# compbioproj-cdna-to-genome-map-align/gmap-2024

Measured on AMD Instinct MI355X. Metric: aligned cDNA reads/sec (2 kb, GRCh38) at 1/2/4/8 MI355X; DP HBM GB/s vs peak, higher is better.
Workload: dtype int32

## Files before the change

gmap-2024_amd/csrc/dp_device.h:

```cpp
#pragma once
#include <hip/hip_runtime.h>
#include <stdint.h>


#include "gmapdp_internal.h"
#include "../../include/gmapdp.h"
#include "me_device.h"

namespace gmapdp {


constexpr int kSent = (int)0x80000000;

__device__ __forceinline__ int dpp_wave_shl1(int x, int fill) {
  return __builtin_amdgcn_update_dpp(fill, x, 0x130, 0xf, 0xf, false);
}
__device__ __forceinline__ int dpp_wave_shl1_zero(int x) {
  return __builtin_amdgcn_update_dpp(0, x, 0x130, 0xf, 0xf, true);
}
__device__ __forceinline__ int dpp_wave_shr1(int x, int fill) {
  return __builtin_amdgcn_update_dpp(fill, x, 0x138, 0xf, 0xf, false);
}
__device__ __forceinline__ int dpp_wave_shr1_zero(int x) {
  return __builtin_amdgcn_update_dpp(0, x, 0x138, 0xf, 0xf, true);
// ... 196 lines not shown
    const int rr = rs - j;
    const int qp = G.qpos(rr);
    const bool good = active && qp >= 0 && gp >= 0;
    const uint64_t mgood = ballot(good);
    if (good) put_pair(out, t.count + lanes_below(mgood, lane), qp, gp, 0, q[rr], '-', ' ', ' ');
    const int nw = __popcll(mgood);
    t.count += nw;
    if (!t.seen) t.lead += nw;
  }
  t.score += kQopen + dist * kQindel;
  t.nopens += 1;
  t.nindels += dist;
}

__device__ __forceinline__ void emit_genomeskip(int lane, int r, int cs, int dist, const Geo& G, bool watson,
                                                uint64_t chroffset, uint64_t chrhigh, const uint32_t* blocks,
                                                uint64_t nwords, gmapdp_pair* out, Tally& t) {
  if (dist >= kMicrointronLength) {
    if (lane == 0) put_pair(out, t.count, -1, -1, dist, ' ', ' ', ' ', ' ');
    t.count += 1;
    t.seen = true;
    return;
  }
  const int qp = G.qpos(r);
  for (int base = 0; base < dist; base += 64) {
    const int j = base + lane;
    const bool active = j < dist;
    const int gp = G.gpos(cs - j);
    const bool good = active && qp >= 0 && gp >= 0;
    const uint64_t mgood = ballot(good);
    if (good) {
      const char c2 = genomic_nt(blocks, nwords, gp, chroffset, chrhigh, watson);
      put_pair(out, t.count + lanes_below(mgood, lane), qp, gp, 0, ' ', '-', c2, c2);
    }
    const int nw = __popcll(mgood);
    t.count += nw;
    if (!t.seen) t.lead += nw;
  }
  t.score += kTopen + dist * kTindel;
  t.nopens += 1;
  t.nindels += dist;
}

__device__ __forceinline__ uint64_t wave_max_u64(uint64_t x) {
#pragma unroll
  for (int off = 32; off >= 1; off >>= 1) {
    const uint64_t y = __shfl_xor(x, off, 64);
    x = y > x ? y : x;
  }
  return x;
}
template <int S>
__device__ __forceinline__ uint64_t seg_max_u64(uint64_t x) {
#pragma unroll
  for (int off = S / 2; off >= 1; off >>= 1) {
    const uint64_t y = __shfl_xor(x, off, 64);
    x = y > x ? y : x;
  }
  return x;
}

struct BridgeCarry {
  const uint8_t* rowdi;
  const uint8_t* coldi;
  const double* rowp;
  const double* colp;
  const int8_t* isc;
  int rdist;
  struct Part* part;
  int* diag;
};
struct Part {
  double p;
  int s;
  int c;
};

__host__ __device__ inline int gg_dir_nhigh(int W) { return W <= 32 ? 0 : W <= 40 ? 1 : W <= 48 ? 2 : 4; }
struct PackedDirs {
  const uint32_t* lo;
  const uint32_t* hi;
  int W, uband, nhigh;
  __device__ uint32_t operator()(int c, int t, int r) const {
    const int k = r - c + uband;
    if (k < 0 || k >= W) return 0u;
    if (k < 32) return (lo[4 * c + t] >> k) & 1u;
    const int b = t * 8 * nhigh + (k - 32);
    return (hi[c * nhigh + (b >> 5)] >> (b & 31)) & 1u;
  }
};

template <int R, bool CARRY, int S = 64, bool PK = (S < 64), bool STORE = false, bool DPK = false, bool NB = false>
__device__ __forceinline__ void fill_band(int lane, int rlen, int glen, int lband, int uband, int open, int ext,
                                          int late, int track, const int8_t* sc, int srow, const uint8_t* gcl,
                                          uint64_t* dirs, const BridgeCarry* bc_, int& bestr, int& bestc,
                                          int gmax = 0, int* smat = nullptr, int* best_score = nullptr) {
  static_assert(S == 64 || (R == 1 && !CARRY), "segmented fills are single-word, no bridge carry");
  static_assert(!STORE || S == 64, "score matrices are stored by whole-wave fills only");
  static_assert(!DPK || (R == 1 && S == 64), "packed direction words: one-word bands");
  static_assert(!NB || S == 64, "narrow-band shifts: whole-wave fills");
  const int lk = (S == 64) ? lane : (lane & (S - 1));
  const int cend = (S == 64) ? glen : gmax;
  const int sat = kNegInf32;
  const int W = lband + uband + 1;
  const int binit = (track == 2) ? kNegInf32 : 0;
  int Hs[R], E[R], bv[R], bcol[R];
#pragma unroll
  for (int i = 0; i < R; i++) {
    const int k = lk * R + i;
    const int r = k - uband;
    int v = kNegInf32;
    if (k < W && r >= 0 && r <= rlen) v = (r == 0) ? 0 : (r <= lband ? open + r * ext : kNegInf32);
    Hs[i] = v;
    E[i] = kNegInf32;
    bv[i] = binit;
    bcol[i] = 0;
  }
  int kext[R];
#pragma unroll
  for (int i = 0; i < R; i++) kext[i] = (lk * R + i) * ext;
  int cs[R], cc[R];
  double cp[R];
#pragma unroll
  for (int i = 0; i < R; i++) {
    cs[i] = 0;
    cc[i] = 0;
    cp[i] = 0.0;
  }
  int rlen1 = rlen + 1;
  uint32_t scb = 0;
  if constexpr (CARRY && PK) {
    scb = (uint32_t)(size_t)(const __attribute__((address_space(3))) int32_t*)reinterpret_cast<const int32_t*>(sc);
    asm volatile("" : "+v"(rlen1), "+v"(scb));
  }
  int rtop_ext = -uband * ext;
  int oce = open;
  int gi_next = (S == 64) ? 0 : gcl[min(1, glen)];
  for (int c = 1; c <= cend; c++) {
    const bool colact = (S == 64) || (c <= glen);
    int gi;
    if constexpr (S == 64) {
      gi = __builtin_amdgcn_readfirstlane(gcl[c]);
    } else {
      gi = gi_next;
      gi_next = gcl[min(c + 1, glen)];
    }
    const int rtop = c - uband;
    const int rlo = rtop < 1 ? 1 : rtop;
    const int rhigh = (c + lband) < rlen ? (c + lband) : rlen;
    rtop_ext += ext;
    oce += ext;
    const int L0 = (c == 1) ? (kNegInf32 - open + 1) : (c <= uband ? oce : kNegInf32);
    const int row0 = (c <= uband) ? oce : kNegInf32;
    const int8_t* scg = PK ? sc : sc + gi * srow;
    const int gi4 = gi << 2;

    int Ein[R], Hin[R];
#pragma unroll
    for (int i = 0; i < R - 1; i++) { Ein[i] = E[i + 1]; Hin[i] = Hs[i + 1]; }
    if constexpr (NB) {
      Ein[R - 1] = dpp_wave_shl1_zero(E[0]);
      Hin[R - 1] = dpp_wave_shl1_zero(Hs[0]);
    } else {
      Ein[R - 1] = seg_shl1<S>(E[0], kNegInf32, lk);
      Hin[R - 1] = seg_shl1<S>(Hs[0], kNegInf32, lk);
    }

    int Hp[R], En[R], A[R];
    bool valid[R], eb[R], hb[R];
#pragma unroll
    for (int i = 0; i < R; i++) {
      const int k = lk * R + i;
      const int r = rtop + k;
      valid[i] = (k < W) & (r >= rlo) & (r <= rhigh) & colact;
      const int rr = (int)min((unsigned)r, (unsigned)rlen1);
      int s;
      if constexpr (!PK) s = scg[rr];
      else if constexpr (CARRY)
        s = __builtin_amdgcn_sbfe(*(const __attribute__((address_space(3))) int32_t*)(size_t)(scb + 4u * (uint32_t)rr),
                                  gi4, 4);
      else s = __builtin_amdgcn_sbfe(reinterpret_cast<const int32_t*>(sc)[rr], gi4, 4);
      const int es = Hin[i] + open;
      eb[i] = Ein[i] > es - late;
      En[i] = max(Ein[i], es) + ext;
      const int dg = Hs[i] + s;
      hb[i] = En[i] > dg - late;
      Hp[i] = max(En[i], dg);
      A[i] = valid[i] ? Hp[i] + open - rtop_ext - kext[i] : kSent;
    }
    int pre[R];
    pre[0] = A[0];
#pragma unroll
    for (int i = 1; i < R; i++) pre[i] = max(pre[i - 1], A[i]);
    const int X = seg_shr1<S>(seg_scan_max<S>(pre[R - 1]), kSent, lk);
    const int init = max(kNegInf32, L0 + open) - ((rtop > 1) ? rtop_ext - ext : 0);
    int F[R], Hun[R];
    bool vb[R];
#pragma unroll
    for (int i = 0; i < R; i++) {
      const int ex = (i == 0) ? X : max(X, pre[i - 1]);
      F[i] = rtop_ext + kext[i] + max(init, ex);
      vb[i] = F[i] > Hp[i] - late;
      Hun[i] = max(F[i], Hp[i]);
    }
    int Fup, Hup;
    if constexpr (S == 64) {
      Fup = dpp_wave_shr1_zero(F[R - 1]);
      Hup = dpp_wave_shr1_zero(Hun[R - 1]);
    } else {
      Fup = seg_shr1<S>(F[R - 1], kNegInf32, lk);
      Hup = seg_shr1<S>(Hun[R - 1], kNegInf32, lk);
    }
    uint64_t mH[R], mV[R], mE[R], mF[R];
#pragma unroll
    for (int i = 0; i < R; i++) {
      const int k = lk * R + i;
      const int r = rtop + k;
      const bool top = r == rlo;
      const int fprev = top ? kNegInf32 : ((i == 0) ? Fup : F[i - 1]);
      const int hprev = top ? L0 : ((i == 0) ? Hup : Hun[i - 1]);
      const bool fb = fprev > hprev + open - late;
      const uint64_t mvalid = ballot(valid[i]);
      mV[i] = ballot(vb[i]) & mvalid;
      mH[i] = ballot(hb[i]) & ~mV[i] & mvalid;
      mE[i] = ballot(eb[i]) & mvalid;
      mF[i] = ballot(fb) & mvalid;
      const int Hc = max(Hun[i], sat);
      if (STORE && valid[i]) smat[(size_t)c * W + k] = Hc;
      Hs[i] = valid[i] ? ((k == 0) ? Hun[i] : Hc) : ((r == 0) ? row0 : kNegInf32);
      E[i] = valid[i] ? En[i] : kNegInf32;
      const bool cand = valid[i] & ((track == 1) | ((track == 2) & (r == rlen))) & (Hc > bv[i] - late);
      bv[i] = cand ? Hc : bv[i];
      bcol[i] = cand ? c : bcol[i];
    }
    if (CARRY) {
      const BridgeCarry& B = *bc_;
      const int cdi = __builtin_amdgcn_readfirstlane(B.coldi[c]);
      const double cpc = B.colp[c];
      int ics[R], icc[R];
      double icp[R];
#pragma unroll
      for (int i = 0; i < R - 1; i++) { ics[i] = cs[i + 1]; icc[i] = cc[i + 1]; icp[i] = cp[i + 1]; }
      ics[R - 1] = dpp_wave_shl1_zero(cs[0]);
      icc[R - 1] = dpp_wave_shl1_zero(cc[0]);
      {
        const int2 v = *reinterpret_cast<const int2*>(&cp[0]);
        int2 w;
        w.x = dpp_wave_shl1_zero(v.x);
        w.y = dpp_wave_shl1_zero(v.y);
        icp[R - 1] = *reinterpret_cast<const double*>(&w);
      }
#pragma unroll
      for (int i = 0; i < R; i++) {
        const int k = lk * R + i;
        const int r = rtop + k;
        const int other = rlen - r;
        const bool inrow = (r >= 1) & (r <= rlen - 1) & (k < W);
        const bool cand = inrow & (k >= 1) & valid[i] & (c <= glen - 2) & (c < B.rdist - other);
        const int Hc = max(Hun[i], sat);
        int s = 0;
        double p = 0.0;
        if (cand) {
          s = B.isc[B.rowdi[other] & cdi] + Hc;
          p = B.rowp[other] + cpc;
        }
        const bool take = cand & ((icc[i] == 0) | (s > ics[i]) | ((s == ics[i]) & (p > icp[i])));
        cs[i] = take ? s : ics[i];
        cc[i] = take ? c + 1 : icc[i];
        cp[i] = take ? p : icp[i];
        if (inrow && k == uband) B.diag[r] = Hc;
        if (inrow && k == 0) {
          B.part[r].s = cs[i];
          B.part[r].c = cc[i] - 1;
          B.part[r].p = cp[i];
        }
      }
    }
#ifdef GMAPDP_GGX_NODIRS
    if (!CARRY)
#endif
    if constexpr (DPK) {
      if (lane == 0) {
        uint32_t* lo = reinterpret_cast<uint32_t*>(dirs);
        *reinterpret_cast<uint4*>(lo + 4 * c) = make_uint4((uint32_t)mH[0], (uint32_t)mV[0], (uint32_t)mE[0], (uint32_t)mF[0]);
        const int nh = gg_dir_nhigh(W);
        uint32_t* hi = lo + 4 * (glen + 1) + nh * c;
        const uint32_t h0 = (uint32_t)(mH[0] >> 32), h1 = (uint32_t)(mV[0] >> 32), h2 = (uint32_t)(mE[0] >> 32),
                       h3 = (uint32_t)(mF[0] >> 32);
        if (nh == 1) {
          hi[0] = (h0 & 0xffu) | ((h1 & 0xffu) << 8) | ((h2 & 0xffu) << 16) | (h3 << 24);
        } else if (nh == 2) {
          *reinterpret_cast<uint2*>(hi) = make_uint2((h0 & 0xffffu) | (h1 << 16), (h2 & 0xffffu) | (h3 << 16));
        } else if (nh == 4) {
          *reinterpret_cast<uint4*>(hi) = make_uint4(h0, h1, h2, h3);
        }
      }
    } else
    if (lane == 0) {
      uint64_t* dcol = dirs + (size_t)c * 4 * R;
#pragma unroll
      for (int i = 0; i < R; i++) {
        dcol[0 * R + i] = mH[i];
        dcol[1 * R + i] = mV[i];
        dcol[2 * R + i] = mE[i];
// ... 157 lines not shown
      bestc = 0;
    } else {
      const uint32_t rk = (uint32_t)(key >> 12) & 4095u, ck = (uint32_t)key & 4095u;
      bestr = late ? (int)rk : 4095 - (int)rk;
      bestc = late ? (int)ck : 4095 - (int)ck;
    }
  } else {
    bestr = rlen;
    bestc = glen;
  }
}

template <int R>
struct RowDirs {
  const uint64_t* dirs;
  int W, uband;
  __device__ uint32_t operator()(int c, int t, int r) const {
    const int k = r - c + uband;
    if (k < 0 || k >= W || r < 0) return 0u;
    return (uint32_t)(dirs[((size_t)c * 4 + t) * R + (r % R)] >> (r / R)) & 1u;
  }
};

template <typename DA, typename QV, typename GV>
__device__ __forceinline__ void traceback_walk(int lane, const DA& dir, int r, int c, const Geo& G, const QV& q,
                                               const QV& quc, const GV& gch, const uint8_t* __restrict__ cons,
                                               bool watson, uint64_t chroffset, uint64_t chrhigh,
                                               const uint32_t* __restrict__ blocks, uint64_t nwords,
                                               gmapdp_pair* out, Tally& t, int mode = 0) {
  while (r > 0 && c > 0) {
    const uint32_t isV = dir(c, 1, r);
    const uint32_t isH = dir(c, 0, r);
    if (!isV && isH) {
      int n = 0;
      for (int base = 0;; base += 64) {
        const int j = base + lane;
        const bool cont = (c - j >= 1) && dir(c - j, 2, r);
        const uint64_t stop = ~ballot(cont);
        if (stop) { n = base + __ffsll((long long)stop) - 1; break; }
      }
      const int dist = n + 1;
      const int c_end = (c - n - 1) > 0 ? (c - n - 1) : 0;
      emit_genomeskip(lane, r, c_end + dist, dist, G, watson, chroffset, chrhigh, blocks, nwords, out, t);
      c = c_end;
    } else if (isV) {
      int n = 0;
      for (int base = 0;; base += 64) {
        const int j = base + lane;
        const bool cont = (r - j >= 1) && dir(c, 3, r - j);
        const uint64_t stop = ~ballot(cont);
        if (stop) { n = base + __ffsll((long long)stop) - 1; break; }
      }
      const int dist = n + 1;
      const int r_end = (r - n - 1) > 0 ? (r - n - 1) : 0;
      emit_queryskip(lane, r_end + dist, c, dist, G, q, out, t);
      r = r_end;
    } else {
      int n = 0;
      for (int base = 0;; base += 64) {
        const int j = base + lane;
        const bool inrange = (c - j >= 1) && (r - j >= 1);
        const bool cont = (j == 0) || (inrange && !dir(c - j, 0, r - j) && !dir(c - j, 1, r - j));
        const uint64_t stop = ~ballot(cont && inrange);
        if (stop) { n = base + __ffsll((long long)stop) - 1; break; }
      }
      emit_diag(lane, r, c, n, G, q, quc, gch, cons, out, t);
      r -= n;
      c -= n;
    }
  }
  if ((r == 0 && c == 0) || (mode == 1 && c == 0) || (mode == 2 && r == 0)) {
  } else if (mode == 2 || (mode == 0 && c == 0)) {
    emit_queryskip(lane, r, 1, r, G, q, out, t);
  } else {
    emit_genomeskip(lane, 1, c, c, G, watson, chroffset, chrhigh, blocks, nwords, out, t);
  }
}

template <int R, typename WORD>
struct BandDirs {
  const WORD* dirs;
  int W, uband, bitoff;
  __device__ uint32_t operator()(int c, int t, int r) const {
    return dir_bit<R, WORD>(dirs, c, t, r - c + uband, W, bitoff);
  }
};

template <int R, typename WORD = uint64_t, typename QV = const char*, typename GV = const char*>
__device__ __forceinline__ void traceback_band(int lane, const WORD* dirs, int W, int uband, int r, int c,
                                               const Geo& G, const QV& q, const QV& quc, const GV& gch,
                                               const uint8_t* __restrict__ cons, bool watson, uint64_t chroffset,
                                               uint64_t chrhigh, const uint32_t* __restrict__ blocks,
                                               uint64_t nwords, gmapdp_pair* out, Tally& t, int bitoff = 0) {
  const BandDirs<R, WORD> d{dirs, W, uband, bitoff};
  traceback_walk(lane, d, r, c, G, q, quc, gch, cons, watson, chroffset, chrhigh, blocks, nwords, out, t);
}

template <typename GV>
__device__ __forceinline__ void emit_genomeskip_seq(int lane, int r, int cs, int dist, const Geo& G, const GV& gch,
                                                    gmapdp_pair* out, Tally& t) {
  if (dist >= kMicrointronLength) {
    if (lane == 0) put_pair(out, t.count, -1, -1, dist, ' ', ' ', ' ', ' ');
    t.count += 1;
    t.seen = true;
    return;
  }
  const int qp = G.qpos(r);
  for (int base = 0; base < dist; base += 64) {
    const int j = base + lane;
    const bool active = j < dist;
    const int gp = G.gpos(cs - j);
    const bool good = active && qp >= 0 && gp >= 0;
    const uint64_t mgood = ballot(good);
    if (good) {
      const char c2 = gch[cs - j];
      put_pair(out, t.count + lanes_below(mgood, lane), qp, gp, 0, ' ', '-', c2, c2);
    }
    const int nw = __popcll(mgood);
    t.count += nw;
    if (!t.seen) t.lead += nw;
  }
  t.score += kTopen + dist * kTindel;
  t.nopens += 1;
  t.nindels += dist;
}

template <typename DA, typename QV, typename GV>
__device__ __forceinline__ void traceback_local(int lane, const DA& dir, int& r, int& c, int endc, int lband,
                                                int uband, const Geo& G, const QV& q, const QV& quc, const GV& gch,
                                                const uint8_t* __restrict__ cons, gmapdp_pair* out, Tally& t) {
  auto gap = [&]() {
    if (r == 0) {
      if (c <= uband) {
        emit_genomeskip_seq(lane, 0, c, c, G, gch, out, t);
        c = 0;
      }
      return;
    }
    if (c == 0) {
      if (r <= lband) {
        emit_queryskip(lane, r, 0, r, G, q, out, t);
        r = 0;
      }
      return;
    }
    const uint32_t isV = dir(c, 1, r);
    const uint32_t isH = dir(c, 0, r);
    if (!isV && isH) {
      int n = 0;
      for (int base = 0;; base += 64) {
        const int j = base + lane;
        const bool cont = (c - j >= 1) && dir(c - j, 2, r);
        const uint64_t stop = ~ballot(cont);
        if (stop) { n = base + __ffsll((long long)stop) - 1; break; }
      }
      const int dist = n + 1;
      const int c_end = (c - n - 1) > 0 ? (c - n - 1) : 0;
      emit_genomeskip_seq(lane, r, c_end + dist, dist, G, gch, out, t);
      c = c_end;
    } else if (isV) {
      int n = 0;
      for (int base = 0;; base += 64) {
        const int j = base + lane;
        const bool cont = (r - j >= 1) && dir(c, 3, r - j);
        const uint64_t stop = ~ballot(cont);
        if (stop) { n = base + __ffsll((long long)stop) - 1; break; }
      }
// ... 150 lines not shown
    if (p < n) {
      const int4 rec = recs[n - 1 - p];
      const bool gap = rec.x == -1 && rec.y == -1;
      const char comp = (char)((rec.w >> 8) & 0xff);
      if (gap) {
      } else if (comp == ' ') {
        delta = kMismatch;
        eval = true;
      } else if (comp == '-') {
        indel = true;
        eval = true;
      } else {
        delta = kMatch;
      }
    }
    const int up = __shfl_up((int)indel, 1, 64);
    const bool before = (lane == 0) ? prev_indel : (up != 0);
    if (indel) delta = before ? kQindel : kQopen + kQindel;
    const int score = carry + wave_scan_add(lane, delta);
    const int hi = max(high, wave_scan_maxi(lane, score));
    if (eval) worst = min(worst, score - hi);
    carry = __shfl(score, 63, 64);
    high = __shfl(hi, 63, 64);
    prev_indel = __shfl((int)indel, 63, 64) != 0;
  }
  return wave_min_i(worst);
}

__device__ __forceinline__ bool lex_better(int s1, double p1, int s2, double p2) {
  return s1 > s2 || (s1 == s2 && p1 > p2);
}

__device__ inline bool gg_simple_wave(int lane, const DevGenomeProblem& P, int pid, const int8_t* __restrict__ sctab,
                               const int8_t* __restrict__ isctab, const uint8_t* __restrict__ cons, const QView& qL,
                               const QView& qucL, const QView& qR, const QView& qucR, const uint8_t* gclL,
                               const uint8_t* gclR, const GClassView& gchL, const GClassView& gchR,
                               const uint8_t* ldi, const uint8_t* rdi, const double* pL, const double* pR,
                               int* diagL, int* diagR, gmapdp_pair* out, gmapdp_genome_result& res,
                               gmapdp_genome_result* __restrict__ results, const uint8_t* __restrict__ ks = nullptr,
                               const double* __restrict__ raw = nullptr, const uint32_t* __restrict__ blocks = nullptr,
                               uint64_t nwords = 0, const double* __restrict__ metab = nullptr) {
  const int rlen = P.rlength;
  const int8_t* sct = sctab + (size_t)P.mismatchtype * 128 * kNClass;
  const int8_t* iscp = isctab + (size_t)P.iclass * 128;
  const bool halfp = P.flags & kGHalf;
  const Geo GL{P.roffset, P.goffsetL, 1};
  const Geo GR{P.roffset + rlen - 1, P.rev_goffsetR, -1};
  int carryL = 0, carryR = 0;
  for (int base = 0; base < rlen; base += 64) {
    const int r = base + lane + 1;
    int vL = 0, vR = 0;
    if (r <= rlen - 1) {
      vL = sct[(uint8_t)(qucL[r] & 127) * kNClass + gclL[r]];
      vR = sct[(uint8_t)(qucR[r] & 127) * kNClass + gclR[r]];
    }
    const int sL = carryL + wave_scan_add(lane, vL), sR = carryR + wave_scan_add(lane, vR);
    if (r <= rlen - 1) {
      diagL[r] = sL;
      diagR[r] = sR;
    }
    carryL = __shfl(sL, 63, 64);
    carryR = __shfl(sR, 63, 64);
  }
  __threadfence_block();
  uint64_t key = 0;
  for (int rL = lane + 1; rL <= rlen - 1; rL += 64) {
    const int rR = rlen - rL;
    const int it = ldi[rL] & rdi[rR];
    const int kl = (ks && ks[rL]) ? kKnownReward : 0, kr = (ks && ks[rlen + 1 + rR]) ? kKnownReward : 0;
    const int score = diagL[rL] + kl + iscp[it] + kr + diagR[rR];
    if ((it != 0 || kl != 0 || kr != 0) && score >= 0) {
      const uint64_t kk = ((uint64_t)(uint32_t)score << 32) | (uint32_t)rL;
      key = kk > key ? kk : key;
    }
  }
  key = wave_max_u64(key);
  if (key == 0) return false;
  const int bestrL = (int)(key & 0xffffffffu), bestscore = (int)(key >> 32), bestrR = rlen - bestrL;
  const int it = ldi[bestrL] & rdi[bestrR];
  const int scoreI = iscp[it];
  res.introntype = it;
  const int finalscore = halfp ? bestscore - scoreI / 2 : bestscore;
  if (finalscore <= 0) return false;
  if (ks) {
    res.left_prob = ks[bestrL] ? 1.0 : raw ? raw[bestrL] : gg_site_prob(P, blocks, nwords, metab, bestrL);
    res.right_prob = ks[rlen + 1 + bestrR] ? 1.0
                   : raw ? raw[P.glengthL + bestrR] : gg_site_prob(P, blocks, nwords, metab, P.glengthL + bestrR);
  } else {
    res.left_prob = pL[bestrL];
    res.right_prob = pR[bestrR];
  }
  if (!(res.left_prob >= 0.90 && res.right_prob >= 0.90)) return false;
  Tally t = {0, 0, 0, 0, 0, 0, 0, false};
  emit_diag(lane, bestrR, bestrR, bestrR, GR, qR, qucR, gchR, cons, out, t);
  const int nR = t.count;
  reverse_records(lane, out, nR);
  const int new_left = P.goffsetL + (bestrL - 1);
  const int new_right = P.rev_goffsetR - (bestrR - 1);
  if (lane == 0) put_pair(out, nR, -1, -1, new_right - new_left - 1, ' ', ' ', ' ', ' ');
  t.count += 1;
  emit_diag(lane, bestrL, bestrL, bestrL, GL, qL, qucL, gchL, cons, out, t);
  if (lane == 0) {
    res.npairs = t.count;
    res.traceback_score = t.nmatches * kMatch + t.nmismatches * kMismatch;
    res.nmatches = t.nmatches;
    res.nmismatches = t.nmismatches;
    res.dynprogindex = P.dynprogindex + (P.dynprogindex > 0 ? 1 : -1);
    res.new_leftgenomepos = new_left;
    res.new_rightgenomepos = res.exonhead = new_right;
    res.gap_index = nR;
    res.gap_queryjump = 0;
    results[pid] = res;
  }
  return true;
}


}
```

gmap-2024_amd/csrc/dp_kernel.hip:

```cpp
#include "dp_device.h"

namespace gmapdp {

#ifdef GMAPDP_OI_TIMING
__device__ unsigned long long g_gg_marks[2][16];
#define GG_MARK(k)                                                          \
  do {                                                                      \
    if (threadIdx.x == 0) {                                                 \
      atomicAdd(&g_gg_marks[0][k], (unsigned long long)wall_clock64());     \
      atomicAdd(&g_gg_marks[1][k], 1ull);                                   \
    }                                                                       \
  } while (0)
#define GG_MARK_TO(a, b) \
  do {                   \
    for (int gk_ = (a); gk_ <= (b); gk_++) GG_MARK(gk_); \
  } while (0)
extern "C" int gmapdp_debug_gg_marks(unsigned long long* out) {
  if (hipMemcpyFromSymbol(out, HIP_SYMBOL(g_gg_marks), sizeof(g_gg_marks)) != hipSuccess) return 1;
  static const unsigned long long zero[2][16] = {};
  return hipMemcpyToSymbol(HIP_SYMBOL(g_gg_marks), zero, sizeof(zero)) != hipSuccess;
}
#else
#define GG_MARK(k) \
  do {             \
// ... 527 lines not shown

#ifdef GMAPDP_GG_PACK_GLOBAL
constexpr bool kGgPackGlobal = true;
#else
constexpr bool kGgPackGlobal = false;
#endif
__host__ __device__ inline ScratchGG scratch_gg(int rlength, int glengthL, int glengthR, int R, bool dirs_lds,
                                                int W = 64) {
  ScratchGG sv;
  size_t off = 0;
  sv.partB = off; off = align16(off + 16u * (size_t)(rlength + 1));
  sv.partC = off; off = align16(off + 16u * (size_t)(rlength + 1));
  sv.diagL = off; off = align16(off + 4u * (size_t)(rlength + 1));
  sv.diagR = off; off = align16(off + 4u * (size_t)(rlength + 1));
  sv.dirsL = sv.dirsR = off;
  if (!dirs_lds) {
    const bool pk = R == 1 && kGgPackGlobal;
    sv.dirsL = off; off = align16(off + (pk ? gg_dirs_bytes_packed(glengthL, W) : gg_dirs_bytes(glengthL, R)));
    sv.dirsR = off; off = align16(off + (pk ? gg_dirs_bytes_packed(glengthR, W) : gg_dirs_bytes(glengthR, R)));
  }
  sv.total = off;
  return sv;
}

#ifdef GMAPDP_GGX_WPE
#define GGX_ATTR __attribute__((amdgpu_waves_per_eu(GMAPDP_GGX_WPE)))
#else
#define GGX_ATTR
#endif
template <int R, bool DIRS_LDS>
__global__ __launch_bounds__(128) GGX_ATTR void gg_kernel(
    const DevGenomeProblem* __restrict__ probs, const int* __restrict__ order,
    const uint32_t* __restrict__ blocks, uint64_t nwords,
    const char* __restrict__ qseq, const char* __restrict__ qseq_uc, const double* __restrict__ sprob,
    const int8_t* __restrict__ sctab, const uint8_t* __restrict__ constab, const int8_t* __restrict__ isctab,
    gmapdp_genome_result* __restrict__ results, gmapdp_pair* __restrict__ pairs,
    unsigned char* __restrict__ gscratch, const uint8_t* __restrict__ known, const double* __restrict__ metab) {
  extern __shared__ __attribute__((aligned(16))) unsigned char smem[];
  const int tid = threadIdx.x;
  const int lane = tid & 63;
  const int wave = __builtin_amdgcn_readfirstlane(tid >> 6);
  const int pid = order[blockIdx.x];
  const DevGenomeProblem P = probs[pid];
  GG_MARK(0);
  const int rlen = P.rlength, gL = P.glengthL, gR = P.glengthR;
  const int flags = P.flags;
  const bool watson = flags & kFWatson;
  const int late = (flags & kFLate) ? 1 : 0;
  const int lband = P.lbandL, ubandL = P.ubandL, ubandR = P.ubandR;
  const int WL = lband + ubandL + 1, WR = lband + ubandR + 1;
  constexpr bool DPK = R == 1 && (DIRS_LDS || kGgPackGlobal);
  const CarveGG cv = carve_gg(rlen, gL, gR, R, DIRS_LDS, WL > WR ? WL : WR);
  const ScratchGG sv = scratch_gg(rlen, gL, gR, R, DIRS_LDS, WL > WR ? WL : WR);
  unsigned char* gbase = gscratch + P.dirs_offset;
  double* pL = reinterpret_cast<double*>(smem + cv.pL);
  double* pR = reinterpret_cast<double*>(smem + cv.pR);
  Part* partB = reinterpret_cast<Part*>(gbase + sv.partB);
  Part* partC = reinterpret_cast<Part*>(gbase + sv.partC);
  int* diagL = reinterpret_cast<int*>(gbase + sv.diagL);
  int* diagR = reinterpret_cast<int*>(gbase + sv.diagR);
  int32_t* scL = reinterpret_cast<int32_t*>(smem + cv.scL);
  int32_t* scR = reinterpret_cast<int32_t*>(smem + cv.scR);
  uint8_t* gclL = reinterpret_cast<uint8_t*>(smem + cv.gclL);
  uint8_t* gclR = reinterpret_cast<uint8_t*>(smem + cv.gclR);
  uint8_t* ldi = reinterpret_cast<uint8_t*>(smem + cv.ldi);
  uint8_t* rdi = reinterpret_cast<uint8_t*>(smem + cv.rdi);
  int8_t* isc = reinterpret_cast<int8_t*>(smem + cv.isc);
  int* done = reinterpret_cast<int*>(smem + cv.flag);
  uint64_t* dirsL = reinterpret_cast<uint64_t*>(DIRS_LDS ? smem + cv.dirsL : gbase + sv.dirsL);
  uint64_t* dirsR = reinterpret_cast<uint64_t*>(DIRS_LDS ? smem + cv.dirsR : gbase + sv.dirsR);
  const QView qL{qseq + P.qbase, 1}, qucL{qseq_uc + P.qbase, 1};
  const QView qR{qseq + P.qbase + rlen - 1, -1}, qucR{qseq_uc + P.qbase + rlen - 1, -1};
  const GClassView gchL{gclL}, gchR{gclR};
  const int8_t* sct = sctab + (size_t)P.mismatchtype * 128 * kNClass;
  const uint8_t* cons = constab + (size_t)P.genestrand * 128 * kNClass;
  gmapdp_pair* out = pairs + P.pair_offset;
  const int rev_roffset = P.roffset + rlen - 1;
  const Geo GL{P.roffset, P.goffsetL, 1};
  const Geo GR{rev_roffset, P.rev_goffsetR, -1};
  const bool halfp = flags & kGHalf;
  const bool kn = flags & kGKnown;
  const uint8_t* kb = kn ? known + P.known_offset : nullptr;

#ifdef GMAPDP_GGX_NOSTAGE
  for (int i = tid; i < rlen + 2; i += 128) scL[i] = scR[i] = 0x123456;
  for (int i = tid; i < gL + 2; i += 128) gclL[i] = i & 3;
  for (int i = tid; i < gR + 2; i += 128) gclR[i] = i & 3;
  for (int i = tid; i < gL; i += 128) pL[i] = 0.1;
  for (int i = tid; i < gR; i += 128) pR[i] = 0.1;
  if (tid < 64) isc[tid] = tid & 7;
  if (tid == 0) *done = 0;
  __syncthreads();
  if (false)
#endif
  for (int i = tid; i < rlen; i += 128) {
    const char c1 = qseq[P.qbase + i];
    const uint64_t row = *reinterpret_cast<const uint64_t*>(sct + (uint8_t)(c1 & 127) * kNClass);
    uint32_t w = 0;
#pragma unroll
    for (int g = 0; g < 6; g++) w |= (uint32_t)((row >> (8 * g)) & 0xfu) << (4 * g);
    scL[i + 1] = (int32_t)w;
    scR[rlen - i] = (int32_t)w;
  }
#ifndef GMAPDP_GGX_NOSTAGE
  if (tid < 2) {
    scL[tid ? rlen + 1 : 0] = 0;
    scR[tid ? rlen + 1 : 0] = 0;
  }
  {
    const int nG = gL + gR;
    for (int b0 = tid; b0 < nG; b0 += 256) {
      uint32_t wf[2], wv[2], bit[2];
      int cls[2];
      double pv[2];
      bool rcv[2];
#pragma unroll
      for (int u = 0; u < 2; u++) {
        const int jj = b0 + 128 * u;
        const bool act = jj < nG;
        const bool rs = jj >= gL;
        const uint32_t i = (uint32_t)(rs ? jj - gL : jj), L = (uint32_t)(rs ? gR : gL);
        const uint64_t pos = rs ? P.segposR : P.segposL, bound = rs ? P.segboundR : P.segboundL;
        const bool left = rs ? (flags & kGSegRLeft) : (flags & kGSegLLeft);
        rcv[u] = rs ? (flags & kGSegRRc) : (flags & kGSegLRc);
        const uint64_t j = rcv[u] ? L - 1u - i : i;
        bool star;
        uint64_t g;
        if (!left) {
          star = pos >= bound || (pos + L >= bound && j + (pos + L - bound) >= L);
          g = pos + j;
        } else {
          star = pos < bound || (pos < bound + L && j < bound + L - pos);
          g = pos - L + j;
        }
        const uint64_t ptr = (g >> 5) * 3u;
        cls[u] = star ? kStar : (ptr + 2 >= nwords ? kN : -1);
        const uint64_t pp = (cls[u] < 0 && act) ? ptr : 0;
        bit[u] = (uint32_t)(g & 31u);
        wf[u] = blocks[pp + 2];
        wv[u] = blocks[pp + (bit[u] < 16 ? 1 : 0)];
        pv[u] = !act ? 0.0 : sprob ? sprob[P.prob_offset + jj] : gg_site_prob(P, blocks, nwords, metab, jj);
        if (kn && act && kb[jj]) pv[u] = 1.0;
      }
#pragma unroll
      for (int u = 0; u < 2; u++) {
        const int jj = b0 + 128 * u;
        if (jj >= nG) continue;
        int c = cls[u];
        if (c < 0) {
          const int x = (int)((wv[u] >> (2u * (bit[u] & 15u))) & 3u);
          c = ((wf[u] >> bit[u]) & 1u) ? kN : (rcv[u] ? 3 - x : x);
        }
        if (jj < gL) {
          gclL[jj + 1] = (uint8_t)c;
          pL[jj] = pv[u];
        } else {
          gclR[gR - (jj - gL)] = (uint8_t)c;
          pR[jj - gL] = pv[u];
        }
      }
    }
  }
  if (tid < 64) isc[tid] = isctab[(size_t)P.iclass * 128 + ((flags & kGFinal) ? 64 : 0) + tid];
  if (tid == 0) *done = 0;
  __syncthreads();
#endif
  for (int c = tid; c <= gL; c += 128) ldi[c] = (c < gL - 1) ? left_dinucl(gchL[c + 1], gchL[c + 2]) : 0;
  for (int c = tid; c <= gR; c += 128) rdi[c] = (c < gR - 1) ? right_dinucl(gchR[c + 2], gchR[c + 1]) : 0;
  __syncthreads();
  GG_MARK(1);

  gmapdp_genome_result res;
  res.npairs = 0;
  res.pair_offset = P.pair_offset;
  res.traceback_score = 0;
  res.nmatches = res.nmismatches = res.nopens = res.nindels = 0;
  res.dynprogindex = P.dynprogindex;
  res.new_leftgenomepos = res.new_rightgenomepos = res.exonhead = kUnset;
  res.introntype = 0;
  res.gap_index = -1;
  res.gap_queryjump = 0;
  res.left_prob = res.right_prob = 0.0;
  const int dpi_next = P.dynprogindex + (P.dynprogindex > 0 ? 1 : -1);

  if (flags & kGSimple) {
    if (wave == 0) {
      const bool ok = gg_simple_wave(lane, P, pid, sctab, isctab, cons, qL, qucL, qR, qucR, gclL, gclR, gchL, gchR,
                                     ldi, rdi, pL, pR, diagL, diagR, out, res, results,
                                     kn ? kb + gL + gR : nullptr, sprob ? sprob + P.prob_offset : nullptr, blocks,
                                     nwords, metab);
      if (lane == 0) *done = ok ? 1 : 0;
    }
    __syncthreads();
    if (*done) {
      GG_MARK_TO(2, 7);
      return;
    }
  }
  GG_MARK(2);

  const int rdist = P.rev_goffsetR - P.goffsetL;
  {
    int br, bc;
    if (wave == 0) {
      const BridgeCarry B{ldi, rdi, pL, pR, isc, rdist, partB, diagR};
      if (WR < 64 * R)
        fill_band<R, true, 64, true, false, DPK, true>(lane, rlen, gR, lband, ubandR, P.open, P.extend, 1 - late, 0,
                                                       reinterpret_cast<const int8_t*>(scR), 0, gclR, dirsR, &B, br,
                                                       bc);
      else
        fill_band<R, true, 64, true, false, DPK>(lane, rlen, gR, lband, ubandR, P.open, P.extend, 1 - late, 0,
                                                 reinterpret_cast<const int8_t*>(scR), 0, gclR, dirsR, &B, br, bc);
    } else {
      const BridgeCarry B{rdi, ldi, pR, pL, isc, rdist, partC, diagL};
      if (WL < 64 * R)
        fill_band<R, true, 64, true, false, DPK, true>(lane, rlen, gL, lband, ubandL, P.open, P.extend, late, 0,
                                                       reinterpret_cast<const int8_t*>(scL), 0, gclL, dirsL, &B, br,
                                                       bc);
      else
        fill_band<R, true, 64, true, false, DPK>(lane, rlen, gL, lband, ubandL, P.open, P.extend, late, 0,
                                                 reinterpret_cast<const int8_t*>(scL), 0, gclL, dirsL, &B, br, bc);
    }
  }
  __threadfence_block();
  __syncthreads();
  GG_MARK(3);
  if (wave != 0) return;
#ifdef GMAPDP_GGX_NOEMIT
  if (lane == 0) results[pid] = res;
  return;
#endif

  int ws = kNegInf32, wrL = -1, wcL = 0, wcR = 0;
  double wp = 0.0;
  int ds = 0, drL = 0x7fffffff;
  double dp = 0.0;
  for (int rL = lane + 1; rL <= rlen - 1; rL += 64) {
    const int rR = rlen - rL;
    const int dL = diagL[rL], dR = diagR[rR];
    const int sI = isc[ldi[rL] & rdi[rR]];
    int rs = dL + sI + dR, rcL = rL, rcR = rR;
    double rp = pL[rL] + pR[rR];
    if (sI > 0 && rp > dp) {
      dp = rp;
      ds = rs;
      drL = rL;
    }
    const Part b = partB[rR];
    if (b.c >= 0 && lex_better(dL + b.s, b.p, rs, rp)) {
      rs = dL + b.s;
      rp = b.p;
      rcL = rL;
      rcR = b.c;
    }
    const Part cpart = partC[rL];
    if (cpart.c >= 0 && lex_better(dR + cpart.s, cpart.p, rs, rp)) {
      rs = dR + cpart.s;
      rp = cpart.p;
      rcL = cpart.c;
      rcR = rR;
    }
    if (lex_better(rs, rp, ws, wp)) {
      ws = rs;
      wp = rp;
      wrL = rL;
      wcL = rcL;
      wcR = rcR;
    }
  }
#pragma unroll
  for (int off = 32; off >= 1; off >>= 1) {
    const int s2 = __shfl_xor(ws, off, 64);
    const double p2 = __shfl_xor(wp, off, 64);
    const int r2 = __shfl_xor(wrL, off, 64);
    const int cl2 = __shfl_xor(wcL, off, 64);
    const int cr2 = __shfl_xor(wcR, off, 64);
    const int ds2 = __shfl_xor(ds, off, 64);
    const double dp2 = __shfl_xor(dp, off, 64);
    const int dr2 = __shfl_xor(drL, off, 64);
    if (lex_better(s2, p2, ws, wp) || (s2 == ws && p2 == wp && r2 < wrL)) {
// ... 248 lines not shown
```

Measured before the change: 350,500.

## Defer score and probability staging to second wave during simple-path attempt

For simple-path problems, staging of query scores and splice-site probabilities is moved out of the common prologue. The second wave now fills them while wave 0 runs the simple bridge, so that work overlaps the simple attempt, and the simple path computes probabilities on demand. Separately, the fill's F-direction bit is now derived from the current row instead of a DPP shift of the previous row, and the traceback readers offset the t==3 bit by one to match. This removes two cross-lane shifts per step but changes the meaning of the direction encoding, which risks correctness if any reader was missed.

```diff
diff --git a/gmap-2024_amd/csrc/dp_device.h b/gmap-2024_amd/csrc/dp_device.h
--- a/gmap-2024_amd/csrc/dp_device.h
+++ b/gmap-2024_amd/csrc/dp_device.h
@@ -302,8 +302,9 @@
   const uint32_t* hi;
   int W, uband, nhigh;
   __device__ uint32_t operator()(int c, int t, int r) const {
-    const int k = r - c + uband;
+    int k = r - c + uband;
     if (k < 0 || k >= W) return 0u;
+    if (t == 3 && --k < 0) return 0u;
     if (k < 32) return (lo[4 * c + t] >> k) & 1u;
     const int b = t * 8 * nhigh + (k - 32);
     return (hi[c * nhigh + (b >> 5)] >> (b & 31)) & 1u;
@@ -423,23 +424,12 @@
       vb[i] = F[i] > Hp[i] - late;
       Hun[i] = max(F[i], Hp[i]);
     }
-    int Fup, Hup;
-    if constexpr (S == 64) {
-      Fup = dpp_wave_shr1_zero(F[R - 1]);
-      Hup = dpp_wave_shr1_zero(Hun[R - 1]);
-    } else {
-      Fup = seg_shr1<S>(F[R - 1], kNegInf32, lk);
-      Hup = seg_shr1<S>(Hun[R - 1], kNegInf32, lk);
-    }
     uint64_t mH[R], mV[R], mE[R], mF[R];
 #pragma unroll
     for (int i = 0; i < R; i++) {
       const int k = lk * R + i;
       const int r = rtop + k;
-      const bool top = r == rlo;
-      const int fprev = top ? kNegInf32 : ((i == 0) ? Fup : F[i - 1]);
-      const int hprev = top ? L0 : ((i == 0) ? Hup : Hun[i - 1]);
-      const bool fb = fprev > hprev + open - late;
+      const bool fb = F[i] > Hun[i] + open - late;
       const uint64_t mvalid = ballot(valid[i]);
       mV[i] = ballot(vb[i]) & mvalid;
       mH[i] = ballot(hb[i]) & ~mV[i] & mvalid;
@@ -763,7 +753,9 @@
   const WORD* dirs;
   int W, uband, bitoff;
   __device__ uint32_t operator()(int c, int t, int r) const {
-    return dir_bit<R, WORD>(dirs, c, t, r - c + uband, W, bitoff);
+    const int k = r - c + uband;
+    if (t == 3) return k < W ? dir_bit<R, WORD>(dirs, c, t, k - 1, W, bitoff) : 0u;
+    return dir_bit<R, WORD>(dirs, c, t, k, W, bitoff);
   }
 };
 
@@ -1080,9 +1072,9 @@
   res.introntype = it;
   const int finalscore = halfp ? bestscore - scoreI / 2 : bestscore;
   if (finalscore <= 0) return false;
-  if (ks) {
-    res.left_prob = ks[bestrL] ? 1.0 : raw ? raw[bestrL] : gg_site_prob(P, blocks, nwords, metab, bestrL);
-    res.right_prob = ks[rlen + 1 + bestrR] ? 1.0
+  if (ks || !pL) {
+    res.left_prob = (ks && ks[bestrL]) ? 1.0 : raw ? raw[bestrL] : gg_site_prob(P, blocks, nwords, metab, bestrL);
+    res.right_prob = (ks && ks[rlen + 1 + bestrR]) ? 1.0
                    : raw ? raw[P.glengthL + bestrR] : gg_site_prob(P, blocks, nwords, metab, P.glengthL + bestrR);
   } else {
     res.left_prob = pL[bestrL];
diff --git a/gmap-2024_amd/csrc/dp_kernel.hip b/gmap-2024_amd/csrc/dp_kernel.hip
--- a/gmap-2024_amd/csrc/dp_kernel.hip
+++ b/gmap-2024_amd/csrc/dp_kernel.hip
@@ -633,6 +633,85 @@
   const bool kn = flags & kGKnown;
   const uint8_t* kb = kn ? known + P.known_offset : nullptr;
 
+  const bool lazy = flags & kGSimple;
+  auto stage_scores = [&](int t0, int nt) __attribute__((always_inline)) {
+    for (int i = t0; i < rlen; i += nt) {
+      const char c1 = qseq[P.qbase + i];
+      const uint64_t row = *reinterpret_cast<const uint64_t*>(sct + (uint8_t)(c1 & 127) * kNClass);
+      uint32_t w = 0;
+#pragma unroll
+      for (int g = 0; g < 6; g++) w |= (uint32_t)((row >> (8 * g)) & 0xfu) << (4 * g);
+      scL[i + 1] = (int32_t)w;
+      scR[rlen - i] = (int32_t)w;
+    }
+    if (t0 < 2) {
+      scL[t0 ? rlen + 1 : 0] = 0;
+      scR[t0 ? rlen + 1 : 0] = 0;
+    }
+  };
+  auto stage_segments = [&](const bool CLS, const bool PRB, int t0, int nt) __attribute__((always_inline)) {
+    const int nG = gL + gR;
+    for (int b0 = t0; b0 < nG; b0 += 2 * nt) {
+      uint32_t wf[2] = {0, 0}, wv[2] = {0, 0}, bit[2] = {0, 0};
+      int cls[2] = {0, 0};
+      double pv[2] = {0.0, 0.0};
+      bool rcv[2] = {false, false};
+#pragma unroll
+      for (int u = 0; u < 2; u++) {
+        const int jj = b0 + nt * u;
+        const bool act = jj < nG;
+        if (CLS) {
+          const bool rs = jj >= gL;
+          const uint32_t i = (uint32_t)(rs ? jj - gL : jj), L = (uint32_t)(rs ? gR : gL);
+          const uint64_t pos = rs ? P.segposR : P.segposL, bound = rs ? P.segboundR : P.segboundL;
+          const bool left = rs ? (flags & kGSegRLeft) : (flags & kGSegLLeft);
+          rcv[u] = rs ? (flags & kGSegRRc) : (flags & kGSegLRc);
+          const uint64_t j = rcv[u] ? L - 1u - i : i;
+          bool star;
+          uint64_t g;
+          if (!left) {
+            star = pos >= bound || (pos + L >= bound && j + (pos + L - bound) >= L);
+            g = pos + j;
+          } else {
+            star = pos < bound || (pos < bound + L && j < bound + L - pos);
+            g = pos - L + j;
+          }
+          const uint64_t ptr = (g >> 5) * 3u;
+          cls[u] = star ? kStar : (ptr + 2 >= nwords ? kN : -1);
+          const uint64_t pp = (cls[u] < 0 && act) ? ptr : 0;
+          bit[u] = (uint32_t)(g & 31u);
+          wf[u] = blocks[pp + 2];
+          wv[u] = blocks[pp + (bit[u] < 16 ? 1 : 0)];
+        }
+        if (PRB) {
+#ifdef GMAPDP_GGX_NOME
+          pv[u] = 0.1;
+#else
+          pv[u] = !act ? 0.0 : sprob ? sprob[P.prob_offset + jj] : gg_site_prob(P, blocks, nwords, metab, jj);
+#endif
+          if (kn && act && kb[jj]) pv[u] = 1.0;
+        }
+      }
+#pragma unroll
+      for (int u = 0; u < 2; u++) {
+        const int jj = b0 + nt * u;
+        if (jj >= nG) continue;
+        if (CLS) {
+          int c = cls[u];
+          if (c < 0) {
+            const int x = (int)((wv[u] >> (2u * (bit[u] & 15u))) & 3u);
+            c = ((wf[u] >> bit[u]) & 1u) ? kN : (rcv[u] ? 3 - x : x);
+          }
+          if (jj < gL) gclL[jj + 1] = (uint8_t)c;
+          else gclR[gR - (jj - gL)] = (uint8_t)c;
+        }
+        if (PRB) {
+          if (jj < gL) pL[jj] = pv[u];
+          else pR[jj - gL] = pv[u];
+        }
+      }
+    }
+  };
 #ifdef GMAPDP_GGX_NOSTAGE
   for (int i = tid; i < rlen + 2; i += 128) scL[i] = scR[i] = 0x123456;
   for (int i = tid; i < gL + 2; i += 128) gclL[i] = i & 3;
@@ -640,82 +719,14 @@
   for (int i = tid; i < gL; i += 128) pL[i] = 0.1;
   for (int i = tid; i < gR; i += 128) pR[i] = 0.1;
   if (tid < 64) isc[tid] = tid & 7;
+#else
+  if (!lazy) stage_scores(tid, 128);
+  if (lazy) stage_segments(true, false, tid, 128);
+  else stage_segments(true, true, tid, 128);
+  if (tid < 64) isc[tid] = isctab[(size_t)P.iclass * 128 + ((flags & kGFinal) ? 64 : 0) + tid];
+#endif
   if (tid == 0) *done = 0;
   __syncthreads();
-  if (false)
-#endif
-  for (int i = tid; i < rlen; i += 128) {
-    const char c1 = qseq[P.qbase + i];
-    const uint64_t row = *reinterpret_cast<const uint64_t*>(sct + (uint8_t)(c1 & 127) * kNClass);
-    uint32_t w = 0;
-#pragma unroll
-    for (int g = 0; g < 6; g++) w |= (uint32_t)((row >> (8 * g)) & 0xfu) << (4 * g);
-    scL[i + 1] = (int32_t)w;
-    scR[rlen - i] = (int32_t)w;
-  }
-#ifndef GMAPDP_GGX_NOSTAGE
-  if (tid < 2) {
-    scL[tid ? rlen + 1 : 0] = 0;
-    scR[tid ? rlen + 1 : 0] = 0;
-  }
-  {
-    const int nG = gL + gR;
-    for (int b0 = tid; b0 < nG; b0 += 256) {
-      uint32_t wf[2], wv[2], bit[2];
-      int cls[2];
-      double pv[2];
-      bool rcv[2];
-#pragma unroll
-      for (int u = 0; u < 2; u++) {
-        const int jj = b0 + 128 * u;
-        const bool act = jj < nG;
-        const bool rs = jj >= gL;
-        const uint32_t i = (uint32_t)(rs ? jj - gL : jj), L = (uint32_t)(rs ? gR : gL);
-        const uint64_t pos = rs ? P.segposR : P.segposL, bound = rs ? P.segboundR : P.segboundL;
-        const bool left = rs ? (flags & kGSegRLeft) : (flags & kGSegLLeft);
-        rcv[u] = rs ? (flags & kGSegRRc) : (flags & kGSegLRc);
-        const uint64_t j = rcv[u] ? L - 1u - i : i;
-        bool star;
-        uint64_t g;
-        if (!left) {
-          star = pos >= bound || (pos + L >= bound && j + (pos + L - bound) >= L);
-          g = pos + j;
-        } else {
-          star = pos < bound || (pos < bound + L && j < bound + L - pos);
-          g = pos - L + j;
-        }
-        const uint64_t ptr = (g >> 5) * 3u;
-        cls[u] = star ? kStar : (ptr + 2 >= nwords ? kN : -1);
-        const uint64_t pp = (cls[u] < 0 && act) ? ptr : 0;
-        bit[u] = (uint32_t)(g & 31u);
-        wf[u] = blocks[pp + 2];
-        wv[u] = blocks[pp + (bit[u] < 16 ? 1 : 0)];
-        pv[u] = !act ? 0.0 : sprob ? sprob[P.prob_offset + jj] : gg_site_prob(P, blocks, nwords, metab, jj);
-        if (kn && act && kb[jj]) pv[u] = 1.0;
-      }
-#pragma unroll
-      for (int u = 0; u < 2; u++) {
-        const int jj = b0 + 128 * u;
-        if (jj >= nG) continue;
-        int c = cls[u];
-        if (c < 0) {
-          const int x = (int)((wv[u] >> (2u * (bit[u] & 15u))) & 3u);
-          c = ((wf[u] >> bit[u]) & 1u) ? kN : (rcv[u] ? 3 - x : x);
-        }
-        if (jj < gL) {
-          gclL[jj + 1] = (uint8_t)c;
-          pL[jj] = pv[u];
-        } else {
-          gclR[gR - (jj - gL)] = (uint8_t)c;
-          pR[jj - gL] = pv[u];
-        }
-      }
-    }
-  }
-  if (tid < 64) isc[tid] = isctab[(size_t)P.iclass * 128 + ((flags & kGFinal) ? 64 : 0) + tid];
-  if (tid == 0) *done = 0;
-  __syncthreads();
-#endif
   for (int c = tid; c <= gL; c += 128) ldi[c] = (c < gL - 1) ? left_dinucl(gchL[c + 1], gchL[c + 2]) : 0;
   for (int c = tid; c <= gR; c += 128) rdi[c] = (c < gR - 1) ? right_dinucl(gchR[c + 2], gchR[c + 1]) : 0;
   __syncthreads();
@@ -734,19 +745,30 @@
   res.left_prob = res.right_prob = 0.0;
   const int dpi_next = P.dynprogindex + (P.dynprogindex > 0 ? 1 : -1);
 
-  if (flags & kGSimple) {
+  if (lazy) {
     if (wave == 0) {
       const bool ok = gg_simple_wave(lane, P, pid, sctab, isctab, cons, qL, qucL, qR, qucR, gclL, gclR, gchL, gchR,
-                                     ldi, rdi, pL, pR, diagL, diagR, out, res, results,
+                                     ldi, rdi, nullptr, nullptr, diagL, diagR, out, res, results,
                                      kn ? kb + gL + gR : nullptr, sprob ? sprob + P.prob_offset : nullptr, blocks,
                                      nwords, metab);
       if (lane == 0) *done = ok ? 1 : 0;
+    } else {
+#ifndef GMAPDP_GGX_NOSTAGE
+      stage_scores(lane, 64);
+#ifndef GMAPDP_GG_PROBS_AFTER_DECLINE
+      stage_segments(false, true, lane, 64);
+#endif
+#endif
     }
     __syncthreads();
     if (*done) {
       GG_MARK_TO(2, 7);
       return;
     }
+#if !defined(GMAPDP_GGX_NOSTAGE) && defined(GMAPDP_GG_PROBS_AFTER_DECLINE)
+    stage_segments(false, true, tid, 128);
+    __syncthreads();
+#endif
   }
   GG_MARK(2);
 
```

Result: faster. 359,600 (median of 6 runs) (+2.6%).
